# pansanity666/TransHuman

Hardware: AMD Instinct MI355X
Metric: rays/sec (512x512, 64 samples/ray) (higher is better)
Workload: dtype f32 (fp16 hi/lo x3 MFMA emulation)

## Files before the change

transhuman_amd/csrc/k_mlp_fused_host.hip:

```cpp
#include <stdio.h>
#include <stdlib.h>
#include <string.h>

#include "k_mlp_fused_kernel.h"
#include "k_mlp_fused8_kernel.h"

__global__ void pack_fused_kernel(const float* __restrict__ W, int N, int K, int KB, int CT, const int* __restrict__ cols,
                                  float scale, uint4* __restrict__ out) {
    long long total = 4LL * KB * CT * 2 * 64;
    for (long long o = blockIdx.x * (long long)blockDim.x + threadIdx.x; o < total;
         o += (long long)gridDim.x * blockDim.x) {
        int lane = (int)(o & 63);
        long long q = o >> 6;
        int plane = (int)(q & 1); q >>= 1;
        int ct = (int)(q % CT); q /= CT;
        int kb = (int)(q % KB);
        int wave = (int)(q / KB);
        int col = cols[wave * CT + ct] + (lane & 31);
        int k0 = 16 * kb + 8 * (lane >> 5);
        h8 v;
#pragma unroll
        for (int j = 0; j < 8; ++j) {
            int k = k0 + j;
            float x = (col < N && k < K) ? W[(long long)col * K + k] * scale : 0.f;
            _Float16 hi, lo;
            split_h(x, hi, lo);
            v[j] = plane == 0 ? hi : lo;
        }
        out[o] = *reinterpret_cast<uint4*>(&v);
    }
}

struct Cols24 { int c[24]; };
__global__ void pack_fused16_kernel(const float* __restrict__ W, int N, int K, int T, int CT, Cols24 cols, float scale, int perm,
                                    uint4* __restrict__ out) {
    long long total = 8LL * T * CT * 2 * 64;
    for (long long o = blockIdx.x * (long long)blockDim.x + threadIdx.x; o < total; o += (long long)gridDim.x * blockDim.x) {
        int lane = (int)(o & 63);
        long long q = o >> 6;
        int plane = (int)(q & 1); q >>= 1;
        int ct = (int)(q % CT); q /= CT;
        int t = (int)(q % T);
        int wave = (int)(q / T);
        int col = cols.c[wave * CT + ct] + (lane & 15);
        int g = lane >> 4;
        int sigma = perm ? 2 * t + (g >> 1) + 16 * (g & 1) : 4 * t + g;
        int k0 = 8 * sigma;
        h8 v;
#pragma unroll
        for (int j = 0; j < 8; ++j) {
            int k = k0 + j;
            float x = (col < N && k < K) ? W[(long long)col * K + k] * scale : 0.f;
            _Float16 hi, lo;
            split_h(x, hi, lo);
            v[j] = plane == 0 ? hi : lo;
        }
        out[o] = *reinterpret_cast<uint4*>(&v);
    }
}

__global__ void absmax_kernel(const float* __restrict__ w, long long n, unsigned int* __restrict__ out) {
    float m = 0.f;
    for (long long i = blockIdx.x * (long long)blockDim.x + threadIdx.x; i < n; i += (long long)gridDim.x * blockDim.x)
        m = fmaxf(m, fabsf(w[i]));
    for (int o = 32; o > 0; o >>= 1) m = fmaxf(m, __shfl_xor(m, o));
    if ((threadIdx.x & 63) == 0) atomicMax(out, __float_as_uint(m));
}

size_t th_fused_pack_bytes() {
    size_t halves = 0;
    const int dims[][2] = {{256, 64},  {256, 384}, {256, 272}, {384, 256}, {384, 256}, {256, 256}, {256, 256},
                           {128, 256}, {128, 32},  {256, 384}, {256, 272}, {128, 128}};
    for (auto& d : dims) halves += (size_t)d[0] * d[1] * 2 + 4096;
    const int dims16[][2] = {{256, 64}, {384, 256}, {384, 256}, {256, 256}, {256, 256}, {128, 256}, {128, 32}, {128, 128}};
    for (auto& d : dims16) halves += (size_t)d[0] * d[1] * 2 + 4096;
    return th_align(halves * 2) + 16 * 256 + 64 * 1024;
}

static int layer_scale_log2(const float* w, long long n, unsigned int* amax_dev, int* out, hipStream_t s) {
    TH_HIP(hipMemsetAsync(amax_dev, 0, 4, s));
    hipLaunchKernelGGL(absmax_kernel, dim3(64), dim3(256), 0, s, w, n, amax_dev);
    unsigned int bits = 0;
    TH_HIP(hipMemcpyAsync(&bits, amax_dev, 4, hipMemcpyDeviceToHost, s));
    TH_HIP(hipStreamSynchronize(s));
    float amax;
    memcpy(&amax, &bits, 4);
    if (!(amax > 0.f) || !(amax < 3.0e38f)) amax = 1.f;
    int e;
    frexpf(amax, &e);
    *out = 13 - e;
    return 0;
}

struct PackCursor {
    char* w;
    float* bias;
    int* cols;
};

static int pack_layer(const float* w, const float* b, int N, int K, int CT, const int* cols_host, int sl2,
                      PackCursor& cur, FusedLayer* out, hipStream_t s) {
    const int KB = (K + 15) / 16;
    if (b) TH_HIP(hipMemcpyAsync(cur.bias, b, (size_t)N * 4, hipMemcpyDeviceToDevice, s));
    else TH_HIP(hipMemsetAsync(cur.bias, 0, (size_t)N * 4, s));
    TH_HIP(hipMemcpyAsync(cur.cols, cols_host, 4 * CT * sizeof(int), hipMemcpyHostToDevice, s));
    uint4* dst = (uint4*)cur.w;
    long long total = 4LL * KB * CT * 2 * 64;
    hipLaunchKernelGGL(pack_fused_kernel, dim3(256), dim3(256), 0, s, w, N, K, KB, CT, cur.cols, ldexpf(1.f, sl2), dst);
    TH_HIP(hipStreamSynchronize(s));
    out->w = dst;
    out->bias = cur.bias;
    out->inv_scale = ldexpf(1.f, -sl2);
    out->CT = CT;
    out->KB = KB;
    cur.w += th_align((size_t)total * 16);
    cur.bias += (N + 3) & ~3;
    cur.cols += 16;
    return 0;
}

static int pack_layer16(const float* w, int N, int K, int CT, const int* cols_host, const FusedLayer& base, int sl2, PackCursor& cur,
                        FusedLayer* out, hipStream_t s) {
    const int T = (K + 31) / 32;
    Cols24 cols{};
    for (int i = 0; i < 8 * CT; ++i) cols.c[i] = cols_host[i];
    uint4* dst = (uint4*)cur.w;
    const long long total = 8LL * T * CT * 2 * 64;
    hipLaunchKernelGGL(pack_fused16_kernel, dim3(256), dim3(256), 0, s, w, N, K, T, CT, cols, ldexpf(1.f, sl2), K == 256 ? 1 : 0, dst);
    TH_LAUNCH_CHECK();
    *out = base;
    out->w = dst;
    out->CT = CT;
    out->KB = T;
    cur.w += th_align((size_t)total * 16);
    return 0;
}

__global__ void fold_matmul_kernel(const float* __restrict__ F, const float* __restrict__ Vw, float* __restrict__ out) {
    int o = blockIdx.x, k = threadIdx.x;
    double acc = 0.0;
    for (int m = 0; m < 256; ++m) acc += (double)F[o * 256 + m] * (double)Vw[m * 256 + k];
    out[o * 256 + k] = (float)acc;
}
__global__ void fold_bias_kernel(const float* __restrict__ F, const float* __restrict__ bF, const float* __restrict__ b1,
                                 const float* __restrict__ b0, float* __restrict__ out) {
    int o = threadIdx.x;
    double acc = bF ? (double)bF[o] : 0.0;
    for (int m = 0; m < 256; ++m) {
        double bm = (b1 ? (double)b1[m] : 0.0) + (b0 ? (double)b0[m] : 0.0);
        acc += (double)F[o * 256 + m] * bm;
    }
    out[o] = (float)acc;
}

__global__ void fold_mm_kernel(const float* __restrict__ A, int lda, const float* __restrict__ B, int ldb, int K, int N,
                               float* __restrict__ out, int ldo) {
    const int m = blockIdx.x;
    for (int n = threadIdx.x; n < N; n += blockDim.x) {
        double acc = 0.0;
        for (int k = 0; k < K; ++k) acc += (double)A[(long long)m * lda + k] * (double)B[(long long)k * ldb + n];
        out[(long long)m * ldo + n] = (float)acc;
    }
}
__global__ void fold_mv_kernel(const float* __restrict__ A, int lda, int K, const float* __restrict__ b0,
                               const float* __restrict__ b1, const float* __restrict__ b2, float* __restrict__ out) {
    const int m = blockIdx.x * blockDim.x + threadIdx.x;
    double acc = b0 ? (double)b0[m] : 0.0;
    for (int k = 0; k < K; ++k)
        acc += (double)A[(long long)m * lda + k] * ((b1 ? (double)b1[k] : 0.0) + (b2 ? (double)b2[k] : 0.0));
    out[m] = (float)acc;
}
__global__ void scale_rows_kernel(const float* __restrict__ src, int lds_, int rows, int cols, float scale,
                                  float* __restrict__ dst, int ldd) {
    long long n = (long long)rows * cols;
    for (long long i = blockIdx.x * (long long)blockDim.x + threadIdx.x; i < n; i += (long long)gridDim.x * blockDim.x) {
        int r = (int)(i / cols), c = (int)(i % cols);
        dst[(long long)r * ldd + c] = src[(long long)r * lds_ + c] * scale;
    }
}

int th_fused_pack(const th_mlp_weights* w, const th_linear* folded, void* store, FusedParams* out, hipStream_t s) {
    char* tail = (char*)store + th_fused_pack_bytes() - 64 * 1024;
    PackCursor cur{(char*)store, (float*)tail, (int*)(tail + 40 * 1024)};
    unsigned int* amax = (unsigned int*)(tail + 60 * 1024);
    int c256[8], c128[4], ckv[12], cst[8];
    int c256_16[16], c128_16[8], ckv16[24];
    for (int wv = 0; wv < 8; ++wv) {
        c256_16[wv * 2] = wv * 32; c256_16[wv * 2 + 1] = wv * 32 + 16;
        c128_16[wv] = wv * 16;
        ckv16[wv * 3] = wv * 16; ckv16[wv * 3 + 1] = 128 + wv * 32; ckv16[wv * 3 + 2] = 128 + wv * 32 + 16;
    }
    for (int wv = 0; wv < 4; ++wv) {
        c256[wv * 2] = wv * 64; c256[wv * 2 + 1] = wv * 64 + 32;
        c128[wv] = wv * 32;
        ckv[wv * 3] = wv * 32; ckv[wv * 3 + 1] = 128 + wv * 64; ckv[wv * 3 + 2] = 128 + wv * 64 + 32;
        cst[wv * 2] = wv * 32; cst[wv * 2 + 1] = 128 + wv * 32;
    }
    int sl2, sl2b;
#define PACK_SIMPLE(LAYER, L, N_, K_, CT_, COLS)                                       \
    TH_TRY(layer_scale_log2((L).w, (long long)(N_) * (K_), amax, &sl2, s));            \
    TH_TRY(pack_layer((L).w, (L).b, N_, K_, CT_, COLS, sl2, cur, &out->LAYER, s))
    float* scratch = nullptr;
    const size_t n_scratch = 256 * 63 + 128 * 256 + 128 * 384 + 128 * 260 + 256 * 384 + 256 + (384 * 256 + 384);
    TH_HIP(hipMalloc((void**)&scratch, n_scratch * 4));
    struct Free { float* p; ~Free() { (void)hipFree(p); } } free_scratch{scratch};
    float* wpe = scratch;
    float* XF = wpe + 256 * 63;
    float* XR = XF + 128 * 256;
    float* XRc = XR + 128 * 384;
    float* st = XRc + 128 * 260;
    float* stb = st + 256 * 384;
    float* tw = stb + 256;
    {
        TH_HIP(hipMemcpy2DAsync(wpe, 63 * 4, w->fc_0.w + 192, 255 * 4, 63 * 4, 256, hipMemcpyDeviceToDevice, s));
        TH_TRY(layer_scale_log2(wpe, 256LL * 63, amax, &sl2, s));
        TH_TRY(pack_layer(wpe, w->fc_0.b, 256, 63, 2, c256, sl2, cur, &out->fc_0pe, s));
        TH_TRY(pack_layer16(wpe, 256, 63, 2, c256_16, out->fc_0pe, sl2, cur, &out->w16.fc_0pe, s));
    }
    PACK_SIMPLE(ar0, w->alpha_res_0, 256, 384, 2, c256);
    PACK_SIMPLE(fc_2, w->fc_2, 256, 256, 2, c256);
    TH_TRY(pack_layer16(w->fc_2.w, 256, 256, 2, c256_16, out->fc_2, sl2, cur, &out->w16.fc_2, s));
    PACK_SIMPLE(fc_3, w->fc_3, 256, 256, 2, c256);
    TH_TRY(pack_layer16(w->fc_3.w, 256, 256, 2, c256_16, out->fc_3, sl2, cur, &out->w16.fc_3, s));
    PACK_SIMPLE(fc_4, w->fc_4, 128, 128, 1, c128);
    TH_TRY(pack_layer16(w->fc_4.w, 128, 128, 1, c128_16, out->fc_4, sl2, cur, &out->w16.fc_4, s));
#undef PACK_SIMPLE
    out->compact_ready = false;
    if (folded) {
        TH_TRY(layer_scale_log2(folded[0].w, 256LL * 260, amax, &sl2, s));
        TH_TRY(pack_layer(folded[0].w, folded[0].b, 256, 260, 2, c256, sl2, cur, &out->ar0c, s));
    }
    {
        const float* Wvf = w->view_fc.w;
        hipLaunchKernelGGL(fold_mm_kernel, dim3(128), dim3(256), 0, s, Wvf, 283, w->feature_fc.w, 256, 256, 256, XF, 256);
        hipLaunchKernelGGL(fold_mm_kernel, dim3(128), dim3(256), 0, s, Wvf, 283, w->rgb_res_0.w, 384, 256, 384, XR, 384);
        if (folded)
            hipLaunchKernelGGL(fold_mm_kernel, dim3(128), dim3(256), 0, s, Wvf, 283, folded[1].w, 260, 256, 260, XRc, 260);
        TH_LAUNCH_CHECK();
        TH_TRY(layer_scale_log2(XF, 128LL * 256, amax, &sl2, s));
        TH_TRY(layer_scale_log2(XR, 128LL * 384, amax, &sl2b, s));
        if (sl2b < sl2) sl2 = sl2b;
        if (folded) {
            TH_TRY(layer_scale_log2(XRc, 128LL * 260, amax, &sl2b, s));
            if (sl2b < sl2) sl2 = sl2b;
        }
        {
            TH_HIP(hipMemcpy2DAsync(st, 27 * 4, Wvf + 256, 283 * 4, 27 * 4, 128, hipMemcpyDeviceToDevice, s));
            TH_TRY(layer_scale_log2(st, 128LL * 27, amax, &sl2b, s));
            if (sl2b < sl2) sl2 = sl2b;
            TH_TRY(pack_layer(st, nullptr, 128, 27, 1, c128, sl2, cur, &out->vfD, s));
            TH_TRY(pack_layer16(st, 128, 27, 1, c128_16, out->vfD, sl2, cur, &out->w16.vfD, s));
        }
        const int s_vf = sl2;
        TH_TRY(pack_layer(XF, nullptr, 128, 256, 1, c128, s_vf, cur, &out->vfA, s));
        TH_TRY(pack_layer16(XF, 128, 256, 1, c128_16, out->vfA, s_vf, cur, &out->w16.vfA, s));
        for (int variant = 0; variant < (folded ? 2 : 1); ++variant) {
            const int K = variant ? 260 : 384;
            const float* xr = variant ? XRc : XR;
            const th_linear& r0 = variant ? folded[1] : w->rgb_res_0;
            const th_linear& r1 = variant ? folded[2] : w->rgb_res_1;
            int s_r1;
            TH_TRY(layer_scale_log2(r1.w, 128LL * K, amax, &s_r1, s));
            hipLaunchKernelGGL(scale_rows_kernel, dim3(128), dim3(256), 0, s, xr, K, 128, K, ldexpf(1.f, s_vf), st, K);
            hipLaunchKernelGGL(scale_rows_kernel, dim3(128), dim3(256), 0, s, r1.w, K, 128, K, ldexpf(1.f, s_r1),
                               st + 128 * K, K);
            hipLaunchKernelGGL(fold_mv_kernel, dim3(1), dim3(128), 0, s, Wvf, 283, 256, w->view_fc.b, w->feature_fc.b,
                               r0.b, stb);
            if (r1.b) TH_HIP(hipMemcpyAsync(stb + 128, r1.b, 128 * 4, hipMemcpyDeviceToDevice, s));
            else TH_HIP(hipMemsetAsync(stb + 128, 0, 128 * 4, s));
            TH_LAUNCH_CHECK();
            FusedLayer* dst = variant ? &out->rstc : &out->rst;
            TH_TRY(pack_layer(st, stb, 256, K, 2, cst, 0, cur, dst, s));
            dst->inv_scale = ldexpf(1.f, -s_vf);
            dst->inv_scale2 = ldexpf(1.f, -s_r1);
        }
        out->vfA.inv_scale = out->vfD.inv_scale = ldexpf(1.f, -s_vf);
        out->compact_ready = folded != nullptr;
    }
    float* tb = tw + 384 * 256;
    for (int which = 0; which < 2; ++which) {
        const th_linear& k = which == 0 ? w->key1 : w->key0;
        const th_linear& v = which == 0 ? w->val1 : w->val0;
        TH_HIP(hipMemcpyAsync(tw, k.w, 128 * 256 * 4, hipMemcpyDeviceToDevice, s));
        hipLaunchKernelGGL(fold_matmul_kernel, dim3(256), dim3(256), 0, s, w->fc_1.w, v.w, tw + 128 * 256);
        if (k.b) TH_HIP(hipMemcpyAsync(tb, k.b, 128 * 4, hipMemcpyDeviceToDevice, s));
        else TH_HIP(hipMemsetAsync(tb, 0, 128 * 4, s));
        TH_HIP(hipMemsetAsync(tb + 128, 0, 256 * 4, s));
        TH_TRY(layer_scale_log2(tw, 384LL * 256, amax, &sl2, s));
        TH_TRY(pack_layer(tw, tb, 384, 256, 3, ckv, sl2, cur, which == 0 ? &out->kv1 : &out->kv0, s));
        TH_TRY(pack_layer16(tw, 384, 256, 3, ckv16, which == 0 ? out->kv1 : out->kv0, sl2, cur, which == 0 ? &out->w16.kv1 : &out->w16.kv0, s));
    }
    hipLaunchKernelGGL(fold_bias_kernel, dim3(1), dim3(256), 0, s, w->fc_1.w, w->fc_1.b, w->val1.b, w->val0.b, cur.bias);
    out->fc_1 = FusedLayer{};
    out->fc_1.bias = cur.bias;
    cur.bias += 256;
    TH_HIP(hipStreamSynchronize(s));
    TH_REQUIRE(cur.w <= tail, "fused pack overflow");
    TH_REQUIRE((char*)cur.bias <= tail + 40 * 1024 && (char*)cur.cols <= tail + 60 * 1024, "fused pack tail overflow");
    return 0;
}

__global__ __launch_bounds__(256) void tok_split_kernel(float* __restrict__ t, int rows, float* __restrict__ sc,
                                                        unsigned int* __restrict__ range) {
    const unsigned bits = reinterpret_cast<const unsigned*>(sc)[1];
    const int E = (int)((bits >> 23) & 255u);
    int sl2 = 0;
    if (E == 255) { if (range != nullptr && blockIdx.x == 0 && threadIdx.x == 0) atomicMax(range + TH_RANGE_VIT, 0x7c00u); }
    else if (bits != 0u) sl2 = min(139 - E, 100);
    const float scale = __builtin_bit_cast(float, (unsigned)(sl2 + 127) << 23);
    if (blockIdx.x == 0 && threadIdx.x == 0) sc[0] = __builtin_bit_cast(float, (unsigned)(127 - sl2) << 23);
    const int lane = threadIdx.x & 63;
    for (int r = blockIdx.x * 4 + (threadIdx.x >> 6); r < rows; r += gridDim.x * 4) {
        float* row = t + (long long)r * 256;
        const float4 x = reinterpret_cast<const float4*>(row)[lane];
        const float v[4] = {x.x * scale, x.y * scale, x.z * scale, x.w * scale};
        h4 hv, lv;
#pragma unroll
        for (int e = 0; e < 4; ++e) {
            _Float16 hi, lo;
            split_h(v[e], hi, lo);
            hv[e] = hi;
            lv[e] = lo;
        }
        __builtin_amdgcn_s_waitcnt(0);
        _Float16* rh = reinterpret_cast<_Float16*>(row);
        *reinterpret_cast<h4*>(rh + 4 * lane) = hv;
        *reinterpret_cast<h4*>(rh + 256 + 4 * lane) = lv;
    }
}

int th_tok_split(float* tprime, int rows, float* sc, unsigned int* range, hipStream_t s) {
    if (rows <= 0) return 0;
    unsigned int* amax = reinterpret_cast<unsigned int*>(sc) + 1;
    TH_HIP(hipMemsetAsync(amax, 0, 4, s));
    hipLaunchKernelGGL(absmax_kernel, dim3(64), dim3(256), 0, s, tprime, (long long)rows * 256, amax);
    hipLaunchKernelGGL(tok_split_kernel, dim3(th_cdiv(rows, 4) < 1024 ? th_cdiv(rows, 4) : 1024), dim3(256), 0, s, tprime, rows, sc,
                       range);
    TH_LAUNCH_CHECK();
    return 0;
}

int th_map_fold_launch(const FusedParams& base, const float* map_split, int V, int H, int W, const int32_t* box, float* fold,
                       unsigned int* range, hipStream_t s, const unsigned* demand) {
    TH_REQUIRE(base.compact_ready, "the map fold needs the colour-folded layers (th_mlp_weights.upsample_color)");
    TH_REQUIRE(V >= 1 && H >= 1 && W >= 1 && map_split && fold, "bad argument");
    MapFoldParams p;
    p.ar0 = base.ar0c; p.rst = base.rstc;
    p.lat = map_split; p.rgb = map_split + (size_t)V * H * W * 256;
    p.box = box; p.V = V; p.H = H; p.W = W;
    p.out0 = fold; p.out12 = fold + (size_t)V * H * W * 256;
    p.range = range;
    p.list = nullptr; p.count = nullptr;
    static unsigned long long attr_done = 0ull;
    if (th_lds_attr_needed(&attr_done)) {
        TH_HIP(hipFuncSetAttribute((const void*)map_fold_kernel<false>, hipFuncAttributeMaxDynamicSharedMemorySize, 2 * MF_TEX * STR272));
        TH_HIP(hipFuncSetAttribute((const void*)map_fold_kernel<true>, hipFuncAttributeMaxDynamicSharedMemorySize, 2 * MF_TEX * STR272));
    }
    if (demand != nullptr) {
        const size_t NW = (size_t)V * H * W / 32;
        p.count = demand + 2 * NW;
        p.list = reinterpret_cast<const int32_t*>(demand + 2 * NW + 16);
        hipLaunchKernelGGL(map_fold_kernel<true>, dim3(512), dim3(256), 2 * MF_TEX * STR272, s, p);
        TH_LAUNCH_CHECK();
        return 0;
    }
    const int tpr = (W + MF_TEX - 1) / MF_TEX;
    hipLaunchKernelGGL(map_fold_kernel<false>, dim3((unsigned)(V * H * tpr)), dim3(256), 2 * MF_TEX * STR272, s, p);
    TH_LAUNCH_CHECK();
    return 0;
}

int th_mlp_fused_forward(const FusedParams& base, const ThMlpPacked& heads, int V, int P, const float* stok,
                         const void* pe, const void* f, int f_ld, const float* vd, const int32_t* vd_sel, int vd_div, int rgb_all, float* raw_c,
                         unsigned int* range, hipStream_t s, const void* tsplit, const float* t_inv, int t_nc, const float* tex_map,
                         size_t tex_stride) {
    if (P <= 0) return 0;
    TH_REQUIRE(V >= 1 && V <= 3, "fused MLP supports 1..3 reference views");
    TH_REQUIRE(f_ld == 384 || (f_ld == 272 && base.compact_ready),
               "pixel-feature rows must be 384 wide, or 272 wide with upsample_color weights uploaded");
    const bool cf = f_ld == 272;
    FusedParams p = base;
    if (cf) { p.ar0 = base.ar0c; p.rst = base.rstc; }
    p.alpha_w = heads.alpha_w; p.alpha_b = heads.alpha_b; p.rgb_w = heads.rgb_w; p.rgb_b = heads.rgb_b;
    TH_REQUIRE(tsplit == nullptr || (t_inv != nullptr && t_nc >= 7 && t_nc <= 4096), "split token table: scale word and 7 <= N_c <= 4096");
    p.tsplit = (const _Float16*)tsplit; p.t_inv = t_inv; p.t_nc = t_nc;
    const bool tex = tex_map != nullptr;
    TH_REQUIRE(!tex || (cf && f != nullptr), "texel hand-over: compact (272-wide) operand planes only");
    p.tex_hdr = nullptr; p.tex_rec = nullptr; p.tex_map = nullptr; p.tex_map2 = nullptr;
    if (tex) {
        p.tex_hdr = (const unsigned*)f;
        p.tex_rec = p.tex_hdr + (size_t)th_cdiv(P, FM_PTS) * 512;
        p.tex_map = tex_map;
        p.tex_map2 = tex_map + tex_stride;
        f = nullptr;
    }
    p.stok = stok; p.pe = (const _Float16*)pe; p.f = (const _Float16*)f; p.vd = vd; p.vd_sel = vd_sel; p.vd_div = vd_div > 0 ? vd_div : 1; p.raw_c = raw_c; p.P = P; p.rgb_all = rgb_all; p.range = range;
    static unsigned long long attr_done = 0ull;
    if (th_lds_attr_needed(&attr_done)) {
#define FM_ATTR(V_, F_)                                                                                       \
    TH_HIP(hipFuncSetAttribute((const void*)mlp_fused_kernel<V_, F_>, hipFuncAttributeMaxDynamicSharedMemorySize, \
                               FUSED_LDS_BYTES))
        FM_ATTR(1, 0); FM_ATTR(2, 0); FM_ATTR(3, 0); FM_ATTR(1, 1); FM_ATTR(2, 1); FM_ATTR(3, 1);
#undef FM_ATTR
#define FM_ATTR_T(V_)                                                                                              \
    TH_HIP(hipFuncSetAttribute((const void*)mlp_fused_kernel<V_, 1, true>, hipFuncAttributeMaxDynamicSharedMemorySize, \
                               FUSED_LDS_BYTES))
        FM_ATTR_T(1); FM_ATTR_T(2); FM_ATTR_T(3);
#undef FM_ATTR_T
    }
    dim3 grid(tex ? 8 * th_cdiv(th_cdiv(P, FM_PTS), 8) : th_cdiv(P, FM_PTS));
    const bool eight = base.waves == 8 && tex && tsplit != nullptr;
    static unsigned long long attr8_done = 0ull;
    if (eight && th_lds_attr_needed(&attr8_done)) {
        TH_HIP(hipFuncSetAttribute((const void*)mlp_fused8_kernel<1>, hipFuncAttributeMaxDynamicSharedMemorySize, F8_LDS_BYTES));
        TH_HIP(hipFuncSetAttribute((const void*)mlp_fused8_kernel<2>, hipFuncAttributeMaxDynamicSharedMemorySize, F8_LDS_BYTES));
        TH_HIP(hipFuncSetAttribute((const void*)mlp_fused8_kernel<3>, hipFuncAttributeMaxDynamicSharedMemorySize, F8_LDS_BYTES));
    }
    static int dbg_state = getenv("TH_FUSED_DBG") ? 1 : 0;
    static long long* dbg_dev = nullptr;
    p.dbg = base.cycles_buf;
    const bool dbg_now = dbg_state == 1 && P >= 4096 && base.cycles_buf == nullptr;
    hipEvent_t dbg_e0 = nullptr, dbg_e1 = nullptr;
    if (dbg_now) {
        if (!dbg_dev) TH_HIP(hipMalloc((void**)&dbg_dev, 64 * sizeof(long long)));
        TH_HIP(hipMemsetAsync(dbg_dev, 0, 64 * sizeof(long long), s));
        p.dbg = dbg_dev;
        TH_HIP(hipEventCreate(&dbg_e0));
        TH_HIP(hipEventCreate(&dbg_e1));
        TH_HIP(hipStreamSynchronize(s));
        TH_HIP(hipEventRecord(dbg_e0, s));
    }
#define FM_LAUNCH(V_, F_) hipLaunchKernelGGL((mlp_fused_kernel<V_, F_>), grid, dim3(256), FUSED_LDS_BYTES, s, p)
#define FM_LAUNCH_T(V_) hipLaunchKernelGGL((mlp_fused_kernel<V_, 1, true>), grid, dim3(256), FUSED_LDS_BYTES, s, p)
#define FM_LAUNCH_8(V_) hipLaunchKernelGGL((mlp_fused8_kernel<V_>), grid, dim3(F8_THREADS), F8_LDS_BYTES, s, p)
    if (eight) {
        if (V == 1) FM_LAUNCH_8(1); else if (V == 2) FM_LAUNCH_8(2); else FM_LAUNCH_8(3);
    } else if (tex) {
        if (V == 1) FM_LAUNCH_T(1); else if (V == 2) FM_LAUNCH_T(2); else FM_LAUNCH_T(3);
    } else
    switch (V * 2 + (cf ? 1 : 0)) {
        case 2: FM_LAUNCH(1, 0); break;
        case 3: FM_LAUNCH(1, 1); break;
        case 4: FM_LAUNCH(2, 0); break;
        case 5: FM_LAUNCH(2, 1); break;
        case 6: FM_LAUNCH(3, 0); break;
        default: FM_LAUNCH(3, 1); break;
    }
#undef FM_LAUNCH
#undef FM_LAUNCH_T
#undef FM_LAUNCH_8
// ... 25 lines not shown
```

transhuman_amd/csrc/k_mlp_fused_kernel.h:

```cpp
#pragma once
#include <hip/hip_fp16.h>

#include <utility>

#include "th_internal.h"

typedef float f32x16 __attribute__((ext_vector_type(16)));
typedef _Float16 h8 __attribute__((ext_vector_type(8)));
typedef _Float16 h4 __attribute__((ext_vector_type(4)));
typedef float f32x4v __attribute__((ext_vector_type(4)));
typedef unsigned fm_u4 __attribute__((ext_vector_type(4)));

#define FM_PTS 32
#define STR272 560
#define STR256 528
#define STR192 400
#define STR128 272
#define STR64 144
#define STRVD 80
#define KSTR 132

#define ABUF_BYTES (2 * 96 * STR272)
#define MBUF_BYTES (96 * KSTR * 4)
#define MISC_FLOATS (9 * 32 + 128 + 4 * 32 * 4 + 8)
// ... 1178 lines not shown
        {
            f32x16 m;
            {
                f32x2 u2[V][8];
#pragma unroll
                for (int r = 0; r < V; ++r)
#pragma unroll
                    for (int q = 0; q < 8; ++q)
                        u2[r][q] = (f32x2){acc2[0][r][2 * q], acc2[0][r][2 * q + 1]} + (f32x2){acc2[1][r][2 * q], acc2[1][r][2 * q + 1]};
#pragma unroll
                for (int r = 1; r < V; ++r)
#pragma unroll
                    for (int q = 0; q < 8; ++q) u2[0][q] = u2[0][q] + u2[r][q];
#pragma unroll
                for (int q = 0; q < 8; ++q) {
                    u2[0][q] = u2[0][q] * (f32x2){inv_v, inv_v};
                    m[2 * q] = u2[0][q][0];
                    m[2 * q + 1] = u2[0][q][1];
                }
            }
            store_tile_h<STR128, false>(m, myrow, wave * 32, f4_hi, f4_lo, lane, rmax);
            range_commit(P.range, TH_RANGE_F4, seen_4, rmax);
        }
        FM_SYNCL();
        f32x16 a4[1][1];
        zero_acc<1, 1>(a4);
        {
            const int aoff4 = (lane & 31) * STR128 + (lane >> 5) * 16;
#pragma unroll
            for (int kb = 0; kb < 8; ++kb) {
                h8 xh4[1], xl4[1];
                load_xfrag<1, STR128, 0>(f4_hi, f4_lo, aoff4, kb, xh4, xl4);
                mfma_kblock<1, 1>(w4[kb], xh4, xl4, a4);
            }
        }
        finish_tile_b<1>(a4[0], b4, P.fc_4.inv_scale, true);
        float s3[3] = {0.f, 0.f, 0.f};
#pragma unroll
        for (int g = 0; g < 4; ++g)
#pragma unroll
            for (int o = 0; o < 3; ++o) {
                s3[o] = fmaf(a4[0][0][4 * g + 0], rw[o][g].x, s3[o]);
                s3[o] = fmaf(a4[0][0][4 * g + 1], rw[o][g].y, s3[o]);
                s3[o] = fmaf(a4[0][0][4 * g + 2], rw[o][g].z, s3[o]);
                s3[o] = fmaf(a4[0][0][4 * g + 3], rw[o][g].w, s3[o]);
            }
#pragma unroll
        for (int o = 0; o < 3; ++o) s3[o] += __shfl_xor(s3[o], 32);
        if (lane < 32) {
            part[(wave * 32 + lane) * 4 + 0] = s3[0];
            part[(wave * 32 + lane) * 4 + 1] = s3[1];
            part[(wave * 32 + lane) * 4 + 2] = s3[2];
        }
        FM_SYNCL();
        if (tid < 32) {
#pragma unroll
            for (int o = 0; o < 3; ++o)
                rgb_out[o] = part[tid * 4 + o] + part[(32 + tid) * 4 + o] + part[(64 + tid) * 4 + o] +
                             part[(96 + tid) * 4 + o] + P.rgb_b[o];
        }
    }
    if (tid < npts)
        *reinterpret_cast<float4*>(P.raw_c + (long long)(pbase + tid) * 4) =
            make_float4(rgb_out[0], rgb_out[1], rgb_out[2], sig[tid]);
    if (FM_DBG_SAMPLED) {
        atomicAdd(reinterpret_cast<unsigned long long*>(P.dbg + 62), (unsigned long long)(clock64() - dbg_t0));
        atomicAdd(reinterpret_cast<unsigned long long*>(P.dbg + 63), (unsigned long long)(wall_clock64() - dbg_w));
    }
}

struct MapFoldParams {
    FusedLayer ar0, rst;
    const float* lat;
    const float* rgb;
    const int32_t* box;
    int V, H, W;
    float* out0;
    float* out12;
    unsigned int* range;
    const int32_t* list;
    const unsigned* count;
};

#define MF_STORE(c) (c)
#define MF_KB 17
#define MF_RT 3
#define MF_TEX (32 * MF_RT)
template <bool LIST>
__global__ __launch_bounds__(256, 1) void map_fold_kernel(MapFoldParams P) {
    extern __shared__ __attribute__((aligned(16))) char lds[];
    char* hi_pl = lds;
    char* lo_pl = lds + MF_TEX * STR272;
    const int tid = threadIdx.x, lane = tid & 63, wave = tid >> 6;
    int xs = 0, x1 = 0;
    long long trow = 0;
    if constexpr (LIST) {
        const int n = (int)*P.count;
        xs = (int)blockIdx.x * MF_TEX;
        x1 = n - 1;
        if (xs > x1) return;
    } else {
    const int tpr = (P.W + MF_TEX - 1) / MF_TEX;
    const int v = blockIdx.x / (P.H * tpr), rem = blockIdx.x - v * (P.H * tpr);
    const int y = rem / tpr, xt = rem - y * tpr;
    int x0 = 0;
    x1 = P.W - 1;
    if (P.box != nullptr) {
        if (y < P.box[4 * v + 1] || y > P.box[4 * v + 3]) return;
        const int32_t* sp = P.box + 4 * P.V + ((long long)v * P.H + y) * 2;
        x0 = sp[0];
        x1 = sp[1];
    }
    xs = x0 + xt * MF_TEX;
    if (xs > x1) return;
    trow = ((long long)v * P.H + y) * P.W;
    }
    auto texel = [&](int x) __attribute__((always_inline)) -> long long {
        if constexpr (LIST) return (long long)P.list[x];
        else return trow + x;
    };
    for (;;) {
    unsigned rmax = 0u;
    const unsigned seen_f = P.range ? P.range[TH_RANGE_F] : 0u;
    {
        const int wv = __builtin_amdgcn_readfirstlane(wave);
#pragma unroll 4
        for (int k = 0; k < MF_TEX / 4; ++k) {
            const int r = wv + 4 * k;
            const long long t = texel(min(xs + r, x1));
            const float4 q = *reinterpret_cast<const float4*>(P.lat + t * 256 + 4 * lane);
            uint2 h, l;
            split_pair(q.x, q.y, h.x, l.x);
            split_pair(q.z, q.w, h.y, l.y);
            range_acc<false>(rmax, h.x);
            range_acc<false>(rmax, h.y);
            *reinterpret_cast<uint2*>(hi_pl + r * STR272 + lane * 8) = h;
            *reinterpret_cast<uint2*>(lo_pl + r * STR272 + lane * 8) = l;
        }
        if (tid < MF_TEX) {
            const long long t = texel(min(xs + tid, x1));
            const float4 c = *reinterpret_cast<const float4*>(P.rgb + t * 4);
            uint4 th = make_uint4(0u, 0u, 0u, 0u), tl = make_uint4(0u, 0u, 0u, 0u);
            split_pair(c.x, c.y, th.x, tl.x);
            split_pair(c.z, 0.f, th.y, tl.y);
            range_acc<false>(rmax, th.x);
            range_acc<false>(rmax, th.y);
            const uint4 z4 = make_uint4(0u, 0u, 0u, 0u);
            *reinterpret_cast<uint4*>(hi_pl + tid * STR272 + 512) = th;
            *reinterpret_cast<uint4*>(hi_pl + tid * STR272 + 528) = z4;
            *reinterpret_cast<uint4*>(lo_pl + tid * STR272 + 512) = tl;
            *reinterpret_cast<uint4*>(lo_pl + tid * STR272 + 528) = z4;
        }
        range_commit(P.range, TH_RANGE_F, seen_f, rmax);
    }
    __syncthreads();
    const int myrow = lane & 31;
    uint4 wk2[FM_RING_D2][2][2];
    f32x16 acc[2][MF_RT];
    gemm_phase_core<MF_RT, 2, STR272, 32 * STR272, FM_RING_D2, true, 3, false>(hi_pl, lo_pl, wslice(P.ar0, wave, 2, 0), MF_KB, lane, acc, wk2);
    {
        const float sc = P.ar0.inv_scale;
#pragma unroll
        for (int r = 0; r < MF_RT; ++r) {
            const int x = xs + r * 32 + myrow;
            if (MF_STORE(x <= x1)) {
                float* o = P.out0 + texel(x) * 256 + wave * 64 + 4 * (lane >> 5);
#pragma unroll
                for (int c = 0; c < 2; ++c)
#pragma unroll
                    for (int g = 0; g < 4; ++g)
                        *reinterpret_cast<float4*>(o + c * 32 + 8 * g) =
                            make_float4(acc[c][r][4 * g] * sc, acc[c][r][4 * g + 1] * sc, acc[c][r][4 * g + 2] * sc, acc[c][r][4 * g + 3] * sc);
            }
        }
    }
    gemm_phase_core<MF_RT, 2, STR272, 32 * STR272, FM_RING_D2, true, 3, false>(hi_pl, lo_pl, wslice(P.rst, wave, 2, 0), MF_KB, lane, acc, wk2);
    {
        const float s0 = P.rst.inv_scale, s1 = P.rst.inv_scale2;
#pragma unroll
        for (int r = 0; r < MF_RT; ++r) {
            const int x = xs + r * 32 + myrow;
            if (MF_STORE(x <= x1)) {
                float* o = P.out12 + texel(x) * 256 + wave * 32 + 4 * (lane >> 5);
#pragma unroll
                for (int g = 0; g < 4; ++g) {
                    *reinterpret_cast<float4*>(o + 8 * g) =
                        make_float4(acc[0][r][4 * g] * s0, acc[0][r][4 * g + 1] * s0, acc[0][r][4 * g + 2] * s0, acc[0][r][4 * g + 3] * s0);
                    *reinterpret_cast<float4*>(o + 128 + 8 * g) =
                        make_float4(acc[1][r][4 * g] * s1, acc[1][r][4 * g + 1] * s1, acc[1][r][4 * g + 2] * s1, acc[1][r][4 * g + 3] * s1);
                }
            }
        }
    }
    if (!LIST) break;
    xs += (int)gridDim.x * MF_TEX;
    if (xs > x1) break;
    __syncthreads();
    }
}
```

transhuman_amd/csrc/th_internal.h:

```cpp
#pragma once
#include <hip/hip_runtime.h>
#include <stdint.h>
#include <stddef.h>
#include <time.h>
#include <string>

#include "transhuman_hip.h"

#define TH_WAVE 64

void th_set_error(const std::string& msg);
#define TH_FAIL(msg)                                                                \
    do {                                                                            \
        th_set_error(std::string(__func__) + ": " + (msg));                         \
        return -1;                                                                  \
    } while (0)
#define TH_REQUIRE(cond, msg)                                                       \
    do {                                                                            \
        if (!(cond)) TH_FAIL(msg);                                                  \
    } while (0)
#define TH_HIP(call)                                                                \
    do {                                                                            \
        hipError_t e__ = (call);                                                    \
        if (e__ != hipSuccess) {                                                    \
// ... 115 lines not shown
    }
}

struct Bilin {
    int i00, i01, i10, i11;
    float w00, w01, w10, w11;
    int x0, y0, x1, y1;
};

__device__ __forceinline__ Bilin th_bilinear_setup(float u, float v, float sx, float sy, int H, int W) {
    float gx = u * sx - 1.0f, gy = v * sy - 1.0f;
    float ix = ((gx + 1.0f) / 2.0f) * (float)(W - 1);
    float iy = ((gy + 1.0f) / 2.0f) * (float)(H - 1);
    ix = fminf(fmaxf(ix, 0.0f), (float)(W - 1));
    iy = fminf(fmaxf(iy, 0.0f), (float)(H - 1));
    float x0 = floorf(ix), y0 = floorf(iy);
    float x1 = x0 + 1.0f, y1 = y0 + 1.0f;
    Bilin b;
    b.w00 = (x1 - ix) * (y1 - iy);
    b.w01 = (ix - x0) * (y1 - iy);
    b.w10 = (x1 - ix) * (iy - y0);
    b.w11 = (ix - x0) * (iy - y0);
    int xi0 = (int)x0, yi0 = (int)y0, xi1 = xi0 + 1, yi1 = yi0 + 1;
    bool bx1 = xi1 <= W - 1, by1 = yi1 <= H - 1;
    if (!bx1) { b.w01 = 0.f; b.w11 = 0.f; xi1 = W - 1; }
    if (!by1) { b.w10 = 0.f; b.w11 = 0.f; yi1 = H - 1; }
    b.i00 = yi0 * W + xi0; b.i01 = yi0 * W + xi1; b.i10 = yi1 * W + xi0; b.i11 = yi1 * W + xi1;
    b.x0 = xi0; b.y0 = yi0; b.x1 = xi1; b.y1 = yi1;
    return b;
}

__device__ __forceinline__ void th_project(const float* __restrict__ cam, float x, float y, float z, float& u,
                                           float& v) {
    float cx = fmaf(cam[2], z, fmaf(cam[1], y, cam[0] * x)) + cam[9];
    float cy = fmaf(cam[5], z, fmaf(cam[4], y, cam[3] * x)) + cam[10];
    float cz = fmaf(cam[8], z, fmaf(cam[7], y, cam[6] * x)) + cam[11];
    const float* K = cam + 12;
    float px = fmaf(K[2], cz, fmaf(K[1], cy, K[0] * cx));
    float py = fmaf(K[5], cz, fmaf(K[4], cy, K[3] * cx));
    float pz = fmaf(K[8], cz, fmaf(K[7], cy, K[6] * cx));
    u = px / pz;
    v = py / pz;
}

#endif

struct ThMlpPacked {
    ThPacked fc_0, alpha_res_0, kv0, kv1, fc_1, fc_2, fc_3, feature_fc, rgb_res_0, view_fc, rgb_res_1, fc_4;
    ThPacked fc_0tok;
    ThPacked alpha_res_0c, rgb_res_0c, rgb_res_1c;
    bool compact_ready = false;
    float *alpha_w = nullptr, *alpha_b = nullptr;
    float *rgb_w = nullptr, *rgb_b = nullptr;
    bool ready = false;
};
struct ThVitBlockPacked {
    float *ln1_w, *ln1_b, *ln2_w, *ln2_b;
    ThPacked qkv, proj, fc1, fc2;
};
struct ThVitPacked {
    int depth = 0, dim = 0, heads = 0;
    ThVitBlockPacked* blocks = nullptr;
    float *norm_w = nullptr, *norm_b = nullptr;
    bool ready = false;
};

struct FusedLayer {
    const uint4* w;
    const float* bias;
    float inv_scale;
    int CT, KB;
    float inv_scale2;
};
struct Fused16 {
    FusedLayer fc_0pe, kv1, kv0, fc_2, fc_3, fc_4, vfA, vfD;
};
struct FusedParams {
    Fused16 w16;
    int waves;
    FusedLayer fc_0pe;
    FusedLayer kv1, ar0, kv0, fc_1, fc_2, fc_3, fc_4;
    FusedLayer vfA, vfD, rst;
    FusedLayer ar0c, rstc;
    bool compact_ready;
    const float *alpha_w, *alpha_b, *rgb_w, *rgb_b;
    const float* stok;
    const _Float16* tsplit;
    const float* t_inv;
    int t_nc;
    const _Float16* pe;
    const _Float16* f;
    const unsigned* tex_hdr;
    const unsigned* tex_rec;
    const float* tex_map;
    const float* tex_map2;
    const float* vd;
    const int32_t* vd_sel;
    int vd_div;
    float* raw_c;
    int P;
    int rgb_all;
    unsigned int* range;
    long long* dbg;
    long long* cycles_buf;
};
enum { TH_RANGE_F = 0, TH_RANGE_S = 1, TH_RANGE_P = 2, TH_RANGE_N = 3, TH_RANGE_INTER = 4, TH_RANGE_F4 = 5, TH_RANGE_CONV = 6,
       TH_RANGE_VIT = 7 };
size_t th_fused_pack_bytes();
int th_fused_pack(const th_mlp_weights* w, const th_linear* folded, void* store, FusedParams* out, hipStream_t s);
int th_mlp_fused_forward(const FusedParams& base, const ThMlpPacked& heads, int V, int P, const float* stok,
                         const void* pe, const void* f, int f_ld, const float* vd, const int32_t* vd_sel, int vd_div, int rgb_all,
                         float* raw_c, unsigned int* range, hipStream_t s, const void* tsplit = nullptr,
                         const float* t_inv = nullptr, int t_nc = 0, const float* tex_map = nullptr, size_t tex_stride = 0);
static inline bool th_lds_attr_needed(unsigned long long* done) {
    int dev = 0;
    if (hipGetDevice(&dev) != hipSuccess || dev < 0 || dev > 63) return true;
    if ((*done >> dev) & 1ull) return false;
    *done |= 1ull << dev;
    return true;
}
int th_map_fold_launch(const FusedParams& base, const float* map_split, int V, int H, int W, const int32_t* box, float* fold,
                       unsigned int* range, hipStream_t s, const unsigned* demand = nullptr );
size_t th_pixtex_bytes(int V, long long P);
int th_pixtex_launch(int V, int H, int W, const ThPointSrc* ps, const int32_t* sel, int P, const float* cams,
                     const float* scale, void* out, hipStream_t s);
int th_tok_split(float* tprime, int rows, float* sc, unsigned int* range, hipStream_t s);

struct th_ctx {
    void* fused_store = nullptr;
    FusedParams fused{};
    bool fused_ready = false;
    int mlp_mode = 1;
    int vit_mode = 1;
    int tok_gather = 1;
    int tex_rows = 1;
    int device = 0;
    void* mlp_store = nullptr;
    void* vit_store = nullptr;
    ThMlpPacked mlp;
    ThVitPacked vit;
    int32_t* host_pinned = nullptr;
    struct Prepass {
        hipEvent_t ev = nullptr;
        const void* ws = nullptr;
        const void* rays = nullptr;
        int R = 0, S = 0;
        bool valid = false;
        hipEvent_t ev2 = nullptr;
        int npre = 0;
        const void* pre_map = nullptr;
        const void* pre_centres = nullptr;
        const void* pre_pool = nullptr;
        const void* grid_centres = nullptr;
        const void* pre_tokens = nullptr;
        const void* demand = nullptr;
        const void* map_done = nullptr;
    };
    static constexpr int kPrepassSlots = 4;
    Prepass prepass[kPrepassSlots];
    int prepass_rr = 0;
    int n_cu = 256;
    const void* map_completed = nullptr;
    const void* map_completed_demand = nullptr;
    hipStream_t aux = nullptr, aux2 = nullptr;
    hipEvent_t aux_fork = nullptr, aux_join = nullptr, aux2_join = nullptr;
    hipEvent_t after_shade = nullptr;
// ... 138 lines not shown
```

Baseline: 19.04 million.

## Rewrite map fold as persistent kernel with register-resident weights and double-buffered LDS

New measurement: 19.06 million (median of 2 runs). Within noise of the previous version (+0.1%).

```diff
diff --git a/transhuman_amd/csrc/k_mlp_fused_host.hip b/transhuman_amd/csrc/k_mlp_fused_host.hip
--- a/transhuman_amd/csrc/k_mlp_fused_host.hip
+++ b/transhuman_amd/csrc/k_mlp_fused_host.hip
@@ -72,7 +72,8 @@
     const int dims[][2] = {{256, 64},  {256, 384}, {256, 272}, {384, 256}, {384, 256}, {256, 256}, {256, 256},
                            {128, 256}, {128, 32},  {256, 384}, {256, 272}, {128, 128}};
     for (auto& d : dims) halves += (size_t)d[0] * d[1] * 2 + 4096;
-    const int dims16[][2] = {{256, 64}, {384, 256}, {384, 256}, {256, 256}, {256, 256}, {128, 256}, {128, 32}, {128, 128}};
+    const int dims16[][2] = {{256, 64}, {384, 256}, {384, 256}, {256, 256}, {256, 256}, {128, 256}, {128, 32}, {128, 128},
+                             {256, 288}, {256, 288}};
     for (auto& d : dims16) halves += (size_t)d[0] * d[1] * 2 + 4096;
     return th_align(halves * 2) + 16 * 256 + 64 * 1024;
 }
@@ -229,6 +230,7 @@
     if (folded) {
         TH_TRY(layer_scale_log2(folded[0].w, 256LL * 260, amax, &sl2, s));
         TH_TRY(pack_layer(folded[0].w, folded[0].b, 256, 260, 2, c256, sl2, cur, &out->ar0c, s));
+        TH_TRY(pack_layer16(folded[0].w, 256, 260, 2, c256_16, out->ar0c, sl2, cur, &out->ar0c16, s));
     }
     {
         const float* Wvf = w->view_fc.w;
@@ -273,6 +275,7 @@
             TH_TRY(pack_layer(st, stb, 256, K, 2, cst, 0, cur, dst, s));
             dst->inv_scale = ldexpf(1.f, -s_vf);
             dst->inv_scale2 = ldexpf(1.f, -s_r1);
+            if (variant) TH_TRY(pack_layer16(st, 256, K, 2, c256_16, *dst, 0, cur, &out->rstc16, s));
         }
         out->vfA.inv_scale = out->vfD.inv_scale = ldexpf(1.f, -s_vf);
         out->compact_ready = folded != nullptr;
@@ -345,7 +348,8 @@
     TH_REQUIRE(base.compact_ready, "the map fold needs the colour-folded layers (th_mlp_weights.upsample_color)");
     TH_REQUIRE(V >= 1 && H >= 1 && W >= 1 && map_split && fold, "bad argument");
     MapFoldParams p;
-    p.ar0 = base.ar0c; p.rst = base.rstc;
+    TH_REQUIRE(base.ar0c16.KB == MF_KS && base.rstc16.KB == MF_KS, "the map fold's weight images have 9 k-steps");
+    p.ar0 = base.ar0c16; p.rst = base.rstc16;
     p.lat = map_split; p.rgb = map_split + (size_t)V * H * W * 256;
     p.box = box; p.V = V; p.H = H; p.W = W;
     p.out0 = fold; p.out12 = fold + (size_t)V * H * W * 256;
@@ -353,19 +357,18 @@
     p.list = nullptr; p.count = nullptr;
     static unsigned long long attr_done = 0ull;
     if (th_lds_attr_needed(&attr_done)) {
-        TH_HIP(hipFuncSetAttribute((const void*)map_fold_kernel<false>, hipFuncAttributeMaxDynamicSharedMemorySize, 2 * MF_TEX * STR272));
-        TH_HIP(hipFuncSetAttribute((const void*)map_fold_kernel<true>, hipFuncAttributeMaxDynamicSharedMemorySize, 2 * MF_TEX * STR272));
+        TH_HIP(hipFuncSetAttribute((const void*)map_fold_kernel<false>, hipFuncAttributeMaxDynamicSharedMemorySize, MF_LDS_BYTES));
+        TH_HIP(hipFuncSetAttribute((const void*)map_fold_kernel<true>, hipFuncAttributeMaxDynamicSharedMemorySize, MF_LDS_BYTES));
     }
     if (demand != nullptr) {
         const size_t NW = (size_t)V * H * W / 32;
         p.count = demand + 2 * NW;
         p.list = reinterpret_cast<const int32_t*>(demand + 2 * NW + 16);
-        hipLaunchKernelGGL(map_fold_kernel<true>, dim3(512), dim3(256), 2 * MF_TEX * STR272, s, p);
+        hipLaunchKernelGGL(map_fold_kernel<true>, dim3(MF_GRID), dim3(MF_THREADS), MF_LDS_BYTES, s, p);
         TH_LAUNCH_CHECK();
         return 0;
     }
-    const int tpr = (W + MF_TEX - 1) / MF_TEX;
-    hipLaunchKernelGGL(map_fold_kernel<false>, dim3((unsigned)(V * H * tpr)), dim3(256), 2 * MF_TEX * STR272, s, p);
+    hipLaunchKernelGGL(map_fold_kernel<false>, dim3(MF_GRID), dim3(MF_THREADS), MF_LDS_BYTES, s, p);
     TH_LAUNCH_CHECK();
     return 0;
 }
diff --git a/transhuman_amd/csrc/k_mlp_fused_kernel.h b/transhuman_amd/csrc/k_mlp_fused_kernel.h
--- a/transhuman_amd/csrc/k_mlp_fused_kernel.h
+++ b/transhuman_amd/csrc/k_mlp_fused_kernel.h
@@ -1284,119 +1284,211 @@
     const unsigned* count;
 };
 
+#ifndef MF_CT
+#define MF_CT 2
+#endif
+#define MF_NS (4 / MF_CT)
+#define MF_T 64
+#define MF_KS 9
+#define MF_STR 592
+#define MF_PLANE (MF_T * MF_STR)
+#define MF_LDS_BYTES (4 * MF_PLANE + 3 * MF_T * 4)
+#define MF_THREADS 512
+#define MF_GRID 256
+static_assert(MF_CT == 1 || MF_CT == 2, "one or two column tiles per wave");
+static_assert(MF_LDS_BYTES <= 163840, "the fold's two operand buffers must fit the CU's LDS");
+static_assert(MF_GRID % (8 * MF_NS) == 0, "whole workers per XCD");
+#ifdef MF_NO_STORE
+#define MF_STORE(c) ((c) && P.V < 0)
+#else
 #define MF_STORE(c) (c)
-#define MF_KB 17
-#define MF_RT 3
-#define MF_TEX (32 * MF_RT)
+#endif
+#ifdef MF_NO_MFMA
+#define MF_MFMA(A, B, C) (C)
+#else
+#define MF_MFMA(A, B, C) __builtin_amdgcn_mfma_f32_16x16x32_f16((A), (B), (C), 0, 0, 0)
+#endif
+
 template <bool LIST>
-__global__ __launch_bounds__(256, 1) void map_fold_kernel(MapFoldParams P) {
+__global__ __launch_bounds__(MF_THREADS, 1) void map_fold_kernel(MapFoldParams P) {
     extern __shared__ __attribute__((aligned(16))) char lds[];
-    char* hi_pl = lds;
-    char* lo_pl = lds + MF_TEX * STR272;
-    const int tid = threadIdx.x, lane = tid & 63, wave = tid >> 6;
-    int xs = 0, x1 = 0;
-    long long trow = 0;
-    if constexpr (LIST) {
-        const int n = (int)*P.count;
-        xs = (int)blockIdx.x * MF_TEX;
-        x1 = n - 1;
-        if (xs > x1) return;
-    } else {
-    const int tpr = (P.W + MF_TEX - 1) / MF_TEX;
-    const int v = blockIdx.x / (P.H * tpr), rem = blockIdx.x - v * (P.H * tpr);
-    const int y = rem / tpr, xt = rem - y * tpr;
-    int x0 = 0;
-    x1 = P.W - 1;
-    if (P.box != nullptr) {
-        if (y < P.box[4 * v + 1] || y > P.box[4 * v + 3]) return;
-        const int32_t* sp = P.box + 4 * P.V + ((long long)v * P.H + y) * 2;
-        x0 = sp[0];
-        x1 = sp[1];
-    }
-    xs = x0 + xt * MF_TEX;
-    if (xs > x1) return;
-    trow = ((long long)v * P.H + y) * P.W;
-    }
-    auto texel = [&](int x) __attribute__((always_inline)) -> long long {
-        if constexpr (LIST) return (long long)P.list[x];
-        else return trow + x;
+    int* tix = reinterpret_cast<int*>(lds + 4 * MF_PLANE);
+    const int tid = threadIdx.x, lane = tid & 63, wave = __builtin_amdgcn_readfirstlane(tid >> 6);
+    const int l15 = lane & 15, g4 = lane >> 4;
+    const int bidx = (int)blockIdx.x >> 3;
+    const int slice = bidx % MF_NS;
+    const int worker = ((int)blockIdx.x & 7) + 8 * (bidx / MF_NS);
+    const int nwork = (int)gridDim.x / MF_NS;
+    const int nrows = P.V * P.H;
+    const int nlist = LIST ? (int)*P.count : 0;
+    int cur = worker, curx = -1;
+    auto fill = [&](int b) __attribute__((always_inline)) -> int {
+        const int slot = tid & (MF_T - 1);
+        int mine = -1, f = 0;
+        if constexpr (LIST) {
+            const long long s0 = (long long)cur * MF_T;
+            const long long left = (long long)nlist - s0;
+            f = left <= 0 ? 0 : (left < MF_T ? (int)left : MF_T);
+            if (slot < f) mine = P.list[s0 + slot];
+            cur += nwork;
+        } else {
+            while (f < MF_T && cur < nrows) {
+                const int v = cur / P.H, y = cur - v * P.H;
+                int x0 = 0, x1 = P.W - 1;
+                if (P.box != nullptr) {
+                    if (y < P.box[4 * v + 1] || y > P.box[4 * v + 3]) x1 = -1;
+                    else {
+                        const int32_t* sp = P.box + 4 * P.V + (long long)cur * 2;
+                        x0 = max(sp[0], 0);
+                        x1 = min(sp[1], P.W - 1);
+                    }
+                }
+                if (curx < x0) curx = x0;
+                const int rem = x1 - curx + 1;
+                if (rem <= 0) { cur += nwork; curx = -1; continue; }
+                const int take = min(rem, MF_T - f);
+                if (slot >= f && slot < f + take) mine = cur * P.W + curx + (slot - f);
+                f += take;
+                curx += take;
+                if (curx > x1) { cur += nwork; curx = -1; }
+            }
+        }
+        if (tid < MF_T) tix[b * MF_T + tid] = mine;
+        return f;
     };
-    for (;;) {
+    int nv = fill(0);
+    if (nv == 0) return;
+    __syncthreads();
+
     unsigned rmax = 0u;
     const unsigned seen_f = P.range ? P.range[TH_RANGE_F] : 0u;
-    {
-        const int wv = __builtin_amdgcn_readfirstlane(wave);
-#pragma unroll 4
-        for (int k = 0; k < MF_TEX / 4; ++k) {
-            const int r = wv + 4 * k;
-            const long long t = texel(min(xs + r, x1));
-            const float4 q = *reinterpret_cast<const float4*>(P.lat + t * 256 + 4 * lane);
+    float4 q[MF_T / 8], qc;
+    auto request = [&](int b) __attribute__((always_inline)) {
+        const int* tx = tix + b * MF_T;
+        const int t0 = tx[0];
+#pragma unroll
+        for (int k = 0; k < MF_T / 8; ++k) {
+            int t = tx[wave + 8 * k];
+            t = t < 0 ? t0 : t;
+            q[k] = *reinterpret_cast<const float4*>(P.lat + (long long)t * 256 + 4 * lane);
+        }
+        if (tid < MF_T) {
+            int t = tx[tid];
+            t = t < 0 ? t0 : t;
+            qc = *reinterpret_cast<const float4*>(P.rgb + (long long)t * 4);
+        }
+    };
+    auto commit = [&](int pb) __attribute__((always_inline)) {
+        char* hi_pl = lds + pb * (2 * MF_PLANE);
+        char* lo_pl = hi_pl + MF_PLANE;
+#pragma unroll
+        for (int k = 0; k < MF_T / 8; ++k) {
+            const int r = wave + 8 * k;
             uint2 h, l;
-            split_pair(q.x, q.y, h.x, l.x);
-            split_pair(q.z, q.w, h.y, l.y);
+            split_pair(q[k].x, q[k].y, h.x, l.x);
+            split_pair(q[k].z, q[k].w, h.y, l.y);
             range_acc<false>(rmax, h.x);
             range_acc<false>(rmax, h.y);
-            *reinterpret_cast<uint2*>(hi_pl + r * STR272 + lane * 8) = h;
-            *reinterpret_cast<uint2*>(lo_pl + r * STR272 + lane * 8) = l;
-        }
-        if (tid < MF_TEX) {
-            const long long t = texel(min(xs + tid, x1));
-            const float4 c = *reinterpret_cast<const float4*>(P.rgb + t * 4);
+            *reinterpret_cast<uint2*>(hi_pl + r * MF_STR + lane * 8) = h;
+            *reinterpret_cast<uint2*>(lo_pl + r * MF_STR + lane * 8) = l;
+        }
+        if (tid < MF_T) {
             uint4 th = make_uint4(0u, 0u, 0u, 0u), tl = make_uint4(0u, 0u, 0u, 0u);
-            split_pair(c.x, c.y, th.x, tl.x);
-            split_pair(c.z, 0.f, th.y, tl.y);
+            split_pair(qc.x, qc.y, th.x, tl.x);
+            split_pair(qc.z, 0.f, th.y, tl.y);
             range_acc<false>(rmax, th.x);
             range_acc<false>(rmax, th.y);
             const uint4 z4 = make_uint4(0u, 0u, 0u, 0u);
-            *reinterpret_cast<uint4*>(hi_pl + tid * STR272 + 512) = th;
-            *reinterpret_cast<uint4*>(hi_pl + tid * STR272 + 528) = z4;
-            *reinterpret_cast<uint4*>(lo_pl + tid * STR272 + 512) = tl;
-            *reinterpret_cast<uint4*>(lo_pl + tid * STR272 + 528) = z4;
-        }
-        range_commit(P.range, TH_RANGE_F, seen_f, rmax);
-    }
+            *reinterpret_cast<uint4*>(hi_pl + tid * MF_STR + 512) = th;
+            *reinterpret_cast<uint4*>(lo_pl + tid * MF_STR + 512) = tl;
+#pragma unroll
+            for (int z = 1; z < 4; ++z) {
+                *reinterpret_cast<uint4*>(hi_pl + tid * MF_STR + 512 + 16 * z) = z4;
+                *reinterpret_cast<uint4*>(lo_pl + tid * MF_STR + 512 + 16 * z) = z4;
+            }
+        }
+    };
+    request(0);
+
+    uint4 w[MF_KS][MF_CT][2];
+    float* obase[MF_CT];
+    float osc[MF_CT];
+#pragma unroll
+    for (int c = 0; c < MF_CT; ++c) {
+        const int col = slice * (128 * MF_CT) + wave * (16 * MF_CT) + 16 * c;
+        const int layer = col >> 8, cl = col & 255, j = cl >> 4;
+        const FusedLayer& L = layer == 0 ? P.ar0 : P.rst;
+        const uint4* wl = L.w + ((long long)(j >> 1) * MF_KS * 2 + (j & 1)) * 128 + lane;
+#pragma unroll
+        for (int t = 0; t < MF_KS; ++t) {
+            w[t][c][0] = wl[t * 256];
+            w[t][c][1] = wl[t * 256 + 64];
+        }
+        obase[c] = (layer == 0 ? P.out0 : P.out12) + cl + 4 * g4;
+        osc[c] = layer == 0 ? P.ar0.inv_scale : (cl < 128 ? P.rst.inv_scale : P.rst.inv_scale2);
+    }
+    int nnext = fill(1);
+    commit(0);
     __syncthreads();
-    const int myrow = lane & 31;
-    uint4 wk2[FM_RING_D2][2][2];
-    f32x16 acc[2][MF_RT];
-    gemm_phase_core<MF_RT, 2, STR272, 32 * STR272, FM_RING_D2, true, 3, false>(hi_pl, lo_pl, wslice(P.ar0, wave, 2, 0), MF_KB, lane, acc, wk2);
-    {
-        const float sc = P.ar0.inv_scale;
-#pragma unroll
-        for (int r = 0; r < MF_RT; ++r) {
-            const int x = xs + r * 32 + myrow;
-            if (MF_STORE(x <= x1)) {
-                float* o = P.out0 + texel(x) * 256 + wave * 64 + 4 * (lane >> 5);
-#pragma unroll
-                for (int c = 0; c < 2; ++c)
-#pragma unroll
-                    for (int g = 0; g < 4; ++g)
-                        *reinterpret_cast<float4*>(o + c * 32 + 8 * g) =
-                            make_float4(acc[c][r][4 * g] * sc, acc[c][r][4 * g + 1] * sc, acc[c][r][4 * g + 2] * sc, acc[c][r][4 * g + 3] * sc);
-            }
-        }
-    }
-    gemm_phase_core<MF_RT, 2, STR272, 32 * STR272, FM_RING_D2, true, 3, false>(hi_pl, lo_pl, wslice(P.rst, wave, 2, 0), MF_KB, lane, acc, wk2);
-    {
-        const float s0 = P.rst.inv_scale, s1 = P.rst.inv_scale2;
-#pragma unroll
-        for (int r = 0; r < MF_RT; ++r) {
-            const int x = xs + r * 32 + myrow;
-            if (MF_STORE(x <= x1)) {
-                float* o = P.out12 + texel(x) * 256 + wave * 32 + 4 * (lane >> 5);
-#pragma unroll
-                for (int g = 0; g < 4; ++g) {
-                    *reinterpret_cast<float4*>(o + 8 * g) =
-                        make_float4(acc[0][r][4 * g] * s0, acc[0][r][4 * g + 1] * s0, acc[0][r][4 * g + 2] * s0, acc[0][r][4 * g + 3] * s0);
-                    *reinterpret_cast<float4*>(o + 128 + 8 * g) =
-                        make_float4(acc[1][r][4 * g] * s1, acc[1][r][4 * g + 1] * s1, acc[1][r][4 * g + 2] * s1, acc[1][r][4 * g + 3] * s1);
-                }
-            }
-        }
-    }
-    if (!LIST) break;
-    xs += (int)gridDim.x * MF_TEX;
-    if (xs > x1) break;
-    __syncthreads();
-    }
-}
+
+    constexpr int NR = 4 / MF_CT;
+    const int aoff = l15 * MF_STR + 16 * g4;
+    int ib = 0, ib1 = 1, ib2 = 2, pb = 0;
+#pragma unroll 1
+    for (;;) {
+        if (nnext > 0) request(ib1);
+        const char* hi_pl = lds + pb * (2 * MF_PLANE);
+        const char* lo_pl = hi_pl + MF_PLANE;
+        const int* tx = tix + ib * MF_T;
+#pragma unroll
+        for (int h = 0; h < MF_T / 16 / NR; ++h) {
+            if (h * NR * 16 >= nv) break;
+            f32x4v acc[MF_CT][NR];
+#pragma unroll
+            for (int t = 0; t < MF_KS; ++t) {
+                h8 xh[NR], xl[NR];
+#pragma unroll
+                for (int r = 0; r < NR; ++r) {
+                    xh[r] = *reinterpret_cast<const h8*>(hi_pl + (h * NR + r) * 16 * MF_STR + aoff + 64 * t);
+                    xl[r] = *reinterpret_cast<const h8*>(lo_pl + (h * NR + r) * 16 * MF_STR + aoff + 64 * t);
+                }
+                const f32x4v zero = {0.f, 0.f, 0.f, 0.f};
+#pragma unroll
+                for (int c = 0; c < MF_CT; ++c)
+#pragma unroll
+                    for (int r = 0; r < NR; ++r)
+                        acc[c][r] = MF_MFMA(*reinterpret_cast<const h8*>(&w[t][c][1]), xh[r], t == 0 ? zero : acc[c][r]);
+#pragma unroll
+                for (int c = 0; c < MF_CT; ++c)
+#pragma unroll
+                    for (int r = 0; r < NR; ++r) acc[c][r] = MF_MFMA(*reinterpret_cast<const h8*>(&w[t][c][0]), xl[r], acc[c][r]);
+#pragma unroll
+                for (int c = 0; c < MF_CT; ++c)
+#pragma unroll
+                    for (int r = 0; r < NR; ++r) acc[c][r] = MF_MFMA(*reinterpret_cast<const h8*>(&w[t][c][0]), xh[r], acc[c][r]);
+            }
+#pragma unroll
+            for (int r = 0; r < NR; ++r) {
+                const int tex = tx[(h * NR + r) * 16 + l15];
+                if (MF_STORE(tex >= 0)) {
+#pragma unroll
+                    for (int c = 0; c < MF_CT; ++c) {
+                        const float sc = osc[c];
+                        *reinterpret_cast<float4*>(obase[c] + (long long)tex * 256) =
+                            make_float4(acc[c][r][0] * sc, acc[c][r][1] * sc, acc[c][r][2] * sc, acc[c][r][3] * sc);
+                    }
+                }
+            }
+        }
+        if (nnext == 0) break;
+        commit(pb ^ 1);
+        const int n2 = fill(ib2);
+        __syncthreads();
+        nv = nnext;
+        nnext = n2;
+        const int i0 = ib;
+        ib = ib1; ib1 = ib2; ib2 = i0;
+        pb ^= 1;
+    }
+    range_commit(P.range, TH_RANGE_F, seen_f, rmax);
+}
diff --git a/transhuman_amd/csrc/th_internal.h b/transhuman_amd/csrc/th_internal.h
--- a/transhuman_amd/csrc/th_internal.h
+++ b/transhuman_amd/csrc/th_internal.h
@@ -221,6 +221,7 @@
     FusedLayer kv1, ar0, kv0, fc_1, fc_2, fc_3, fc_4;
     FusedLayer vfA, vfD, rst;
     FusedLayer ar0c, rstc;
+    FusedLayer ar0c16, rstc16;
     bool compact_ready;
     const float *alpha_w, *alpha_b, *rgb_w, *rgb_b;
     const float* stok;
```
